# xitorch/xitorch

Measured on AMD Instinct MI355X. Metric: eigpairs/sec of symeig(davidson) + Lanczos-role matvec GB/s (roofline.achieved), batch=64 N=16384, higher is better.
Workload: dtype f64

## Files before the change

include/xitorch_amd.h:

```cpp
#ifndef XITORCH_AMD_H
#define XITORCH_AMD_H

#ifdef __cplusplus
extern "C" {
#endif

#define XK_OK 0
#define XK_ERR_ARG (-1)
#define XK_ERR_UNSUPPORTED (-2)

int xk_abi_version(void);

int xk_stream_read(const void* src, long bytes, long pitch_bytes, void* scratch, void* stream);
int xk_stream_create_cu_masked(int device, int reserve_cus, void** stream_out);
int xk_stream_create_cu_masked_pattern(int device, int reserve_cus, int pattern, void** stream_out);
int xk_probe_xcc(unsigned* hist16, unsigned* units128, int workgroups, int spin_cycles, void* stream);
int xk_stream_destroy(void* stream);

long xk_dense_mm_workspace_elems(int B, int M, int N, int P, int trans);
int xk_dense_mm_f64(const double* A, const double* X, double* Y, double* ws, long ws_elems,
                    int B, int M, int N, int P, long lda, long sA, long ldx, long sX,
                    long ldy, long sY, int trans, int rows_hint, int stagger, void* stream);
int xk_dense_mm_f32(const float* A, const float* X, float* Y, float* ws, long ws_elems,
                    int B, int M, int N, int P, long lda, long sA, long ldx, long sX,
// ... 2 lines not shown
long xk_dense_symm_workspace_elems(int B, int N, int P, int elem_size);
int xk_dense_symm_f64(const double* A, const double* X, double* Y, double* ws, long ws_elems, int B,
                      int N, int P, long lda, long sA, long ldx, long sX, long ldy, long sY, int opts, void* stream);
int xk_dense_symm_f32(const float* A, const float* X, float* Y, float* ws, long ws_elems, int B, int N,
                      int P, long lda, long sA, long ldx, long sX, long ldy, long sY, int opts, void* stream);
int xk_dense_symm_tiles_f64(const double* A, const double* X, double* ws, long ws_elems, int B, int N, int P,
                            long lda, long sA, long ldx, long sX, int opts, void* stream);
int xk_dense_symm_tiles_f32(const float* A, const float* X, float* ws, long ws_elems, int B, int N, int P,
                            long lda, long sA, long ldx, long sX, int opts, void* stream);
int xk_dense_symm_fold_f64(double* Y, const double* ws, long ws_elems, int B, int N, int P, long ldy, long sY,
                           int opts, void* stream);
int xk_dense_symm_fold_f32(float* Y, const float* ws, long ws_elems, int B, int N, int P, long ldy, long sY,
                           int opts, void* stream);

long xk_dense_symm_wide_workspace_elems(int B, int N);
int xk_dense_symm_wide_f32(const float* A, const float* X, float* Y, float* ws, long ws_elems, int B, int N, int P,
                           long lda, long sA, long ldx, long sX, long ldy, long sY, int opts, void* stream);
int xk_dense_symm_wide_tiles_f32(const float* A, const float* X, float* ws, long ws_elems, int B, int N, int P,
                                 long lda, long sA, long ldx, long sX, int opts, void* stream);
int xk_dense_symm_wide_fold_f32(float* Y, const float* ws, long ws_elems, int B, int N, int P, long ldy, long sY,
                                int opts, void* stream);

long xk_dense_wide_workspace_elems(int B, int M, int N, int P, int elem_size);
int xk_dense_wide_padded_width(int P, int elem_size);
int xk_dense_wide_f32(const float* A, const float* Xrm, float* Y, float* ws, long ws_elems, int B, int M,
                      int N, int P, long lda, long sA, long ldxr, long sXr, long ldy, long sY, void* stream);
int xk_dense_wide_f64(const double* A, const double* Xrm, double* Y, double* ws, long ws_elems, int B, int M,
                      int N, int P, long lda, long sA, long ldxr, long sXr, long ldy, long sY, void* stream);

long xk_dense_rows_wide_workspace_elems(int B, int M, int N, int P, int elem_size);
int xk_dense_rows_wide_f64(const double* A, const double* X, double* Y, double* ws, long ws_elems, int B, int M,
                           int N, int P, long lda, long sA, long ldx, long sX, long ldy, long sY, void* stream);
int xk_dense_rows_wide_f32(const float* A, const float* X, float* Y, float* ws, long ws_elems, int B, int M, int N,
                           int P, long lda, long sA, long ldx, long sX, long ldy, long sY, void* stream);

int xk_lincomb_f64(const double* V, const double* C, double* Out, int B, int k, int N, int P,
                   long ldv, long sV, long sC, long sCa, long sCc, long ldo, long sO,
                   double alpha, double beta, void* stream);
int xk_lincomb_f32(const float* V, const float* C, float* Out, int B, int k, int N, int P,
                   long ldv, long sV, long sC, long sCa, long sCc, long ldo, long sO,
                   double alpha, double beta, void* stream);
int xk_ritz_residual_f64(const double* V, const double* AV, const double* Y, const double* lam,
                         double* X, double* Tn, double* rmax, int B, int k, int N, int P,
                         long ldv, long sV, long ldav, long sAV, long sY, long sYa, long sYc,
                         long sLam, long ldx, long sX, long ldt, long sT, void* stream);
int xk_ritz_residual_f32(const float* V, const float* AV, const float* Y, const float* lam,
                         float* X, float* Tn, float* rmax, int B, int k, int N, int P,
                         long ldv, long sV, long ldav, long sAV, long sY, long sYa, long sYc,
                         long sLam, long ldx, long sX, long ldt, long sT, void* stream);
int xk_panel_chol_f64(const double* G, double* W, int* info, int B, int P, long ldg, long sG, void* stream);
int xk_panel_chol_f32(const float* G, float* W, int* info, int B, int P, long ldg, long sG, void* stream);
int xk_panel_transform_f64(double* Tp, const double* W, int B, int P, int N, long ldt, long sT, void* stream);
int xk_panel_transform_f32(float* Tp, const float* W, int B, int P, int N, long ldt, long sT, void* stream);

int xk_diag_precond_f64(double* t, const double* d, const double* m, const double* lam, int B, int N, int P,
                        long ldt, long sT, long sD, long sM, long sLam, double floor_, void* stream);
int xk_diag_precond_f32(float* t, const float* d, const float* m, const float* lam, int B, int N, int P,
                        long ldt, long sT, long sD, long sM, long sLam, double floor_, void* stream);

int xk_group_status_f64(const double* rmax, const int* info, const int* flag, double* orth, double* status, int B,
                        void* stream);
int xk_group_status_f32(const float* rmax, const int* info, const int* flag, float* orth, double* status, int B,
                        void* stream);

long xk_small_eigh_workspace_elems(int B, int k, int max_sweeps);
int xk_small_eigh_f64(const double* T, double* lam, double* Y, double* ws, long ws_elems, int* sweeps,
                      int B, int k, int p, int uppest, int max_sweeps, long ldt, long sT, void* stream);
int xk_small_eigh_f32(const float* T, float* lam, float* Y, float* ws, long ws_elems, int* sweeps,
                      int B, int k, int p, int uppest, int max_sweeps, long ldt, long sT, void* stream);

long xk_small_eigh_tri_lds_bytes(int k, int p, int elem_size);
int xk_small_eigh_tri_f64(const double* T, double* lam, double* Y, int* info, int B, int k, int p, int uppest,
                          long ldt, long sT, int threads, long long* profile, void* stream);
int xk_small_eigh_tri_f32(const float* T, float* lam, float* Y, int* info, int B, int k, int p, int uppest, long ldt,
                          long sT, int threads, long long* profile, void* stream);

int xk_banded_mm_f64(const double* band, const double* X, double* Y, int B, int N, int hb, int C,
                     long sBand, long ldx, long sX, long ldy, long sY, int trans, void* stream);
int xk_banded_mm_f32(const float* band, const float* X, float* Y, int B, int N, int hb, int C,
                     long sBand, long ldx, long sX, long ldy, long sY, int trans, void* stream);

int xk_csr_seg_len(void);
int xk_csr_mm_f64(const int* ptr, const int* idx, const int* perm, const double* val, long sV, const int* rows,
                  const int* bin_off, const int* seg_q, const int* seg_off, int nseg, double* ws, const double* X,
                  double* Y, int B, int Mout, int Nin, int C, long ldx, long sX, long ldy, long sY, void* stream);
int xk_csr_mm_f32(const int* ptr, const int* idx, const int* perm, const float* val, long sV, const int* rows,
                  const int* bin_off, const int* seg_q, const int* seg_off, int nseg, float* ws, const float* X,
                  float* Y, int B, int Mout, int Nin, int C, long ldx, long sX, long ldy, long sY, void* stream);
int xk_csr_sddmm_f64(const int* row_of, const int* col, const double* U, const double* W, double* G, int nnz, int B,
                     int M, int N, int C, long ldu, long sU, long ldw, long sW, long sG, void* stream);
int xk_csr_sddmm_f32(const int* row_of, const int* col, const float* U, const float* W, float* G, int nnz, int B,
                     int M, int N, int C, long ldu, long sU, long ldw, long sW, long sG, void* stream);
int xk_csr_mm_c128(const int* ptr, const int* idx, const int* perm, const double* val, long sV, const int* rows,
                   const int* bin_off, const int* seg_q, const int* seg_off, int nseg, double* ws, const double* X,
                   double* Y, int B, int Mout, int Nin, int C, long ldx, long sX, long ldy, long sY, int conj_val,
                   void* stream);
int xk_csr_mm_c64(const int* ptr, const int* idx, const int* perm, const float* val, long sV, const int* rows,
                  const int* bin_off, const int* seg_q, const int* seg_off, int nseg, float* ws, const float* X,
                  float* Y, int B, int Mout, int Nin, int C, long ldx, long sX, long ldy, long sY, int conj_val,
                  void* stream);
int xk_csr_sddmm_c128(const int* row_of, const int* col, const double* U, const double* W, double* G, int nnz, int B,
                      int M, int N, int C, long ldu, long sU, long ldw, long sW, long sG, void* stream);
int xk_csr_sddmm_c64(const int* row_of, const int* col, const float* U, const float* W, float* G, int nnz, int B,
                     int M, int N, int C, long ldu, long sU, long ldw, long sW, long sG, void* stream);

int xk_banded_grad_f64(const double* U, const double* W, double* G, int B, int N, int hb, int C, long ldu,
// ... 298 lines not shown
```

xitorch_amd/csrc/xk_basis.hip:

```cpp
#include "xk_common.h"

namespace xk {

template <typename T, int P>
__global__ __launch_bounds__(256) void lincomb_kernel(
    const T* __restrict__ V, const T* __restrict__ C, T* __restrict__ Out,
    int k, int N, long ldv, long sV, long sC, long sCa, long sCc, long ldo, long sO,
    T alpha, T beta, int col_tiles) {
  typedef typename Vec16<T>::type VT;
  constexpr int VN = Vec16<T>::n;
  const int b = blockIdx.x / col_tiles;
  const int ct = blockIdx.x - b * col_tiles;
  const int j = (ct * 256 + threadIdx.x) * VN;
  if (j >= N) return;
  const T* Vb = V + (long)b * sV + j;
  const T* Cb = C + (long)b * sC;
  VT acc[P];
#pragma unroll
  for (int c = 0; c < P; ++c)
#pragma unroll
    for (int v = 0; v < VN; ++v) acc[c][v] = T(0);
  int a = 0;
  for (; a + 8 <= k; a += 8) {
    VT v[8];
// ... 235 lines not shown
  constexpr int VN = Vec16<T>::n;
  if (!vec_ok<T>(N, ldv, sV, V) || !vec_ok<T>(N, ldo, sO, Out)) return XK_ERR_UNSUPPORTED;
  const int ct = (N + 256 * VN - 1) / (256 * VN);
  int c0 = 0;
  while (c0 < P) {
    const int pc = (P - c0) >= 8 ? 8 : (P - c0);
    const T* Cc = C + (long)c0 * sCc;
    T* Oc = Out + (long)c0 * ldo;
    switch (pc) {
#define XK_CASE(PP)                                                                                   \
  case PP:                                                                                            \
    hipLaunchKernelGGL((lincomb_kernel<T, PP>), dim3((unsigned)((long)B * ct)), dim3(256), 0, st, V, \
                       Cc, Oc, k, N, ldv, sV, sC, sCa, sCc, ldo, sO, alpha, beta, ct);                \
    break;
      XK_CASE(1) XK_CASE(2) XK_CASE(3) XK_CASE(4) XK_CASE(5) XK_CASE(6) XK_CASE(7) XK_CASE(8)
#undef XK_CASE
    }
    XK_LAUNCH_CHECK();
    c0 += pc;
  }
  return XK_OK;
}

template <typename T>
static int ritz_residual(const T* V, const T* AV, const T* Y, const T* lam, T* X, T* Tn, T* rmax, int B,
                         int k, int N, int P, long ldv, long sV, long ldav, long sAV, long sY, long sYa,
                         long sYc, long sLam, long ldx, long sX, long ldt, long sT, hipStream_t st) {
  constexpr int VN = Vec16<T>::n;
  if (!vec_ok<T>(N, ldv, sV, V) || !vec_ok<T>(N, ldav, sAV, AV) || !vec_ok<T>(N, ldx, sX, X) ||
      !vec_ok<T>(N, ldt, sT, Tn))
    return XK_ERR_UNSUPPORTED;
  const int ct = (N + 256 * VN - 1) / (256 * VN);
  int c0 = 0;
  while (c0 < P) {
    const int pc = (P - c0) >= 8 ? 8 : (P - c0);
    switch (pc) {
#define XK_CASE(PP)                                                                                    \
  case PP:                                                                                             \
    hipLaunchKernelGGL((ritz_residual_kernel<T, PP>), dim3((unsigned)((long)B * ct)), dim3(256), 0,   \
                       st, V, AV, Y + (long)c0 * sYc, lam + c0, X + (long)c0 * ldx, Tn + (long)c0 * ldt, \
                       rmax, k, N, ldv, sV, ldav, sAV, sY, sYa, sYc, sLam, ldx, sX, ldt, sT, ct);       \
    break;
      XK_CASE(1) XK_CASE(2) XK_CASE(3) XK_CASE(4) XK_CASE(5) XK_CASE(6) XK_CASE(7) XK_CASE(8)
#undef XK_CASE
    }
    XK_LAUNCH_CHECK();
    c0 += pc;
  }
  return XK_OK;
}


template <typename T>
__global__ __launch_bounds__(256) void diag_precond_kernel(T* __restrict__ Tn, const T* __restrict__ d,
                                                            const T* __restrict__ m, const T* __restrict__ lam,
                                                            int N, int P, long ldt, long sT, long sD, long sM,
                                                            long sLam, T floor_, long total) {
  const long idx = (long)blockIdx.x * 256 + threadIdx.x;
  if (idx >= total) return;
  const long per_b = (long)P * N;
  const long b = idx / per_b;
  const long rem = idx - b * per_b;
  const int c = (int)(rem / N);
  const int n = (int)(rem - (long)c * N);
  const T mm = m ? m[b * sM + n] : T(1);
  T den = d[b * sD + n] - lam[b * sLam + c] * mm;
  if (fabs(den) < floor_) den = den < T(0) ? -floor_ : floor_;
  T* t = Tn + b * sT + (long)c * ldt + n;
  *t = *t / den;
}

template <typename T>
__global__ __launch_bounds__(64) void group_status_kernel(const T* __restrict__ rmax, const int* __restrict__ info,
                                                          const int* __restrict__ flag, T* __restrict__ orth,
                                                          double* __restrict__ status, int B) {
  const int lane = threadIdx.x;
  double m = 0.0, om_ = 0.0;
  int nan = 0, i1 = 0, i2 = 0;
  bool first = true;
  for (int b = lane; b < B; b += 64) {
    const double v = (double)rmax[b];
    nan |= (v != v);
    m = first ? v : (v > m ? v : m);
    const int a = info[b];
    i1 = first ? a : (a > i1 ? a : i1);
    if (flag) {
      const int f = flag[b];
      i2 = first ? f : (f > i2 ? f : i2);
    }
    if (orth) {
      const double ov = (double)orth[b];
      orth[b] = T(0);
      om_ = (ov != ov) ? __builtin_inf() : (ov > om_ ? ov : om_);
    }
    first = false;
  }
  double mm = first ? -__builtin_inf() : m;
  int a1 = first ? -2147483647 - 1 : i1, a2 = first ? -2147483647 - 1 : i2;
#pragma unroll
  for (int sft = 32; sft >= 1; sft >>= 1) {
    const double om = __shfl_xor(mm, sft, 64), oo = __shfl_xor(om_, sft, 64);
    const int o1 = __shfl_xor(a1, sft, 64), o2 = __shfl_xor(a2, sft, 64), on = __shfl_xor(nan, sft, 64);
    mm = om > mm ? om : mm;
    om_ = oo > om_ ? oo : om_;
    a1 = o1 > a1 ? o1 : a1;
    a2 = o2 > a2 ? o2 : a2;
    nan |= on;
  }
  if (lane == 0) {
    status[0] = nan ? __builtin_nan("") : mm;
    status[1] = (double)a1;
    status[2] = flag ? (double)a2 : 0.0;
    if (orth) status[4] = om_;
  }
}

}

extern "C" {

#define XK_DEFINE_BASIS(SUF, T)                                                                          \
  int xk_lincomb_##SUF(const T* V, const T* C, T* Out, int B, int k, int N, int P, long ldv, long sV,    \
                       long sC, long sCa, long sCc, long ldo, long sO, double alpha, double beta,        \
                       void* stream) {                                                                   \
    if (B < 0 || k < 0 || N < 0 || P < 0) return XK_ERR_ARG;                                             \
    if (B == 0 || N == 0 || P == 0) return XK_OK;                                                        \
    return xk::lincomb<T>(V, C, Out, B, k, N, P, ldv, sV, sC, sCa, sCc, ldo, sO, (T)alpha, (T)beta,      \
                          (hipStream_t)stream);                                                          \
  }                                                                                                      \
  int xk_ritz_residual_##SUF(const T* V, const T* AV, const T* Y, const T* lam, T* X, T* Tn, T* rmax,    \
                             int B, int k, int N, int P, long ldv, long sV, long ldav, long sAV,         \
                             long sY, long sYa, long sYc, long sLam, long ldx, long sX, long ldt,        \
                             long sT, void* stream) {                                                    \
    if (B < 0 || k < 0 || N < 0 || P < 0) return XK_ERR_ARG;                                             \
    if (B == 0 || N == 0 || P == 0) return XK_OK;                                                        \
    return xk::ritz_residual<T>(V, AV, Y, lam, X, Tn, rmax, B, k, N, P, ldv, sV, ldav, sAV, sY, sYa,     \
                                sYc, sLam, ldx, sX, ldt, sT, (hipStream_t)stream);                       \
  }                                                                                                      \
  int xk_panel_chol_##SUF(const T* G, T* W, int* info, int B, int P, long ldg, long sG, void* stream) {  \
    if (B < 0 || P < 0 || P > 32) return XK_ERR_ARG;                                                     \
    if (B == 0 || P == 0) return XK_OK;                                                                  \
    hipLaunchKernelGGL((xk::panel_chol_kernel<T>), dim3((unsigned)B), dim3(64), 0,                       \
                       (hipStream_t)stream, G, W, info, B, P, ldg, sG, (long)P * P);                     \
    XK_LAUNCH_CHECK();                                                                                   \
    return XK_OK;                                                                                        \
  }                                                                                                      \
  int xk_panel_transform_##SUF(T* Tp, const T* W, int B, int P, int N, long ldt, long sT,                \
                               void* stream) {                                                           \
    if (B < 0 || P < 0 || N < 0) return XK_ERR_ARG;                                                      \
    if (B == 0 || P == 0 || N == 0) return XK_OK;                                                        \
    if (!xk::vec_ok<T>(N, ldt, sT, Tp)) return XK_ERR_UNSUPPORTED;                                       \
    constexpr int VN = xk::Vec16<T>::n;                                                                  \
    const int ct = (N + 256 * VN - 1) / (256 * VN);                                                      \
    hipLaunchKernelGGL((xk::panel_transform_kernel<T>), dim3((unsigned)((long)B * ct)), dim3(256), 0,    \
                       (hipStream_t)stream, Tp, W, P, N, ldt, sT, (long)P * P, ct);                      \
    XK_LAUNCH_CHECK();                                                                                   \
    return XK_OK;                                                                                        \
  }

XK_DEFINE_BASIS(f64, double)
XK_DEFINE_BASIS(f32, float)

#define XK_DEFINE_STATUS(SUF, T)                                                                            \
  int xk_group_status_##SUF(const T* rmax, const int* info, const int* flag, T* orth, double* status, int B, \
                            void* stream) {                                                                 \
    if (B <= 0 || !rmax || !info || !status) return XK_ERR_ARG;                                             \
    hipLaunchKernelGGL((xk::group_status_kernel<T>), dim3(1), dim3(64), 0, (hipStream_t)stream, rmax, info, \
                       flag, orth, status, B);                                                              \
    XK_LAUNCH_CHECK();                                                                                      \
    return XK_OK;                                                                                           \
  }
XK_DEFINE_STATUS(f64, double)
XK_DEFINE_STATUS(f32, float)

// ... 16 lines not shown
```

xitorch_amd/kernels.py:

```python
import os
import torch
from xitorch_amd import _capi
from xitorch_amd._capi import ptr, stream_ptr, check, suffix, fn, call, require_device
from ctypes import c_void_p as c_void_p_

__all__ = ["dense_mm"]


def _panel_strides(X):
    if X.dim() != 3 or (X.shape[-1] > 1 and X.stride(-1) != 1):
        raise _capi.NativeLibraryError("panel must be (B, P, N) with unit stride along N, got shape %s stride %s"
                                       % (tuple(X.shape), X.stride()))
    return X.stride(1), X.stride(0)


def _op_strides(A):
    if A.dim() == 2:
        return A.stride(0), 0
    return A.stride(1), (A.stride(0) if A.shape[0] != 1 else 0)


def _esize(dtype):
    return 8 if dtype == torch.float64 else 4

# ... 129 lines not shown
_gs_cache = {}


def _guard_scratch(B, P, dtype, device):
    key = (dtype, device, torch.cuda.current_stream().cuda_stream)
    g = _gs_cache.get(key)
    if g is None or g.numel() < B * P * P:
        g = _gs_cache[key] = torch.empty(B * P * P, dtype=dtype, device=device)
    return g


def _check_ritz_shapes(V, AV, Y, lam, X, Tn, k, P):
    B = V.shape[0]
    if Y.dim() != 3 or Y.shape[0] != B or Y.shape[1] < k or Y.shape[2] < P or lam.shape[0] != B or lam.shape[-1] < P:
        raise _capi.NativeLibraryError("ritz_residual: Y must be (B, >=k, >=P) and lam (B, >=P); got %s / %s for "
                                       "k = %d, P = %d" % (tuple(Y.shape), tuple(lam.shape), k, P))
    if V.shape[1] < k or AV.shape[1] < k or X.shape[1] < P or Tn.shape[1] < P:
        raise _capi.NativeLibraryError("ritz_residual: basis / output panels are smaller than (k, P) = (%d, %d)" % (k, P))


def ritz_residual(V, AV, Y, lam, X, Tn, rmax, k, P):
    B, N = V.shape[0], V.shape[2]
    if lam.stride(-1) != 1 and P > 1:
        raise _capi.NativeLibraryError("lam must have unit stride along its last dim")
    _check_ritz_shapes(V, AV, Y, lam, X, Tn, k, P)
    call("xk_ritz_residual", V.dtype, ptr(V), ptr(AV), ptr(Y), ptr(lam), ptr(X), ptr(Tn), ptr(rmax), B, k, N, P,
         V.stride(1), V.stride(0), AV.stride(1), AV.stride(0), Y.stride(0), Y.stride(1), Y.stride(2), lam.stride(0),
         X.stride(1), X.stride(0), Tn.stride(1), Tn.stride(0))


def diag_precond(Tn, d, lam, P, m=None, floor=None):
    B, N = Tn.shape[0], d.shape[-1]
    if floor is None:
        floor = float(torch.finfo(Tn.dtype).eps) ** 0.5
    d2 = d.reshape(-1, N)
    m2 = m.reshape(-1, N) if m is not None else None
    for t in (d2, m2):
        if t is not None and (t.stride(-1) != 1 or t.dtype != Tn.dtype or t.shape[0] not in (1, B)):
            raise _capi.NativeLibraryError("diag_precond: diagonals must be (B or 1, N), unit stride, dtype of the panel")
    sD = d2.stride(0) if d2.shape[0] == B and B > 1 else (0 if d2.shape[0] == 1 else d2.stride(0))
    sM = 0 if m2 is None or m2.shape[0] == 1 else m2.stride(0)
    call("xk_diag_precond", Tn.dtype, ptr(Tn), ptr(d2), ptr(m2) if m2 is not None else None, ptr(lam), B, N, P,
         Tn.stride(1), Tn.stride(0), sD, sM, lam.stride(0), float(floor))


def panel_chol(G, W, info, P):
    B = G.shape[0]
    call("xk_panel_chol", G.dtype, ptr(G), ptr(W), ptr(info), B, P, G.stride(1), G.stride(0))


def panel_transform(Tp, W, P):
    B, N = Tp.shape[0], Tp.shape[2]
    call("xk_panel_transform", Tp.dtype, ptr(Tp), ptr(W), B, P, N, Tp.stride(1), Tp.stride(0))


def davidson_ritz(V, AV, Y, lam, X, Tn, rmax, info, flag, status, k, P, cond=None, orth=None):
    B, N = V.shape[0], V.shape[2]
    if lam.stride(-1) != 1 and P > 1:
        raise _capi.NativeLibraryError("lam must have unit stride along its last dim")
    _check_ritz_shapes(V, AV, Y, lam, X, Tn, k, P)
    gs, ws, nws = None, None, 0
    if orth is not None:
        if status.numel() < 5:
            raise _capi.NativeLibraryError("davidson_ritz: status needs 5 doubles when orth is given")
        if P > 8:
            gs = _guard_scratch(B, P, V.dtype, V.device)
            nws = fn("xk_dense_mm_workspace_elems")(B, P, N, P, 0)
            ws = _workspace(max(nws, 1), V.dtype, V.device)
    call("xk_davidson_ritz", V.dtype, ptr(V), ptr(AV), ptr(Y), ptr(lam), ptr(X), ptr(Tn), ptr(rmax), ptr(info),
         ptr(flag) if flag is not None else None, ptr(cond) if cond is not None else None,
         ptr(orth) if orth is not None else None, ptr(status), B, k, N, P, V.stride(1), V.stride(0), AV.stride(1),
         AV.stride(0), Y.stride(0), Y.stride(1), Y.stride(2), lam.stride(0), X.stride(1), X.stride(0), Tn.stride(1),
         Tn.stride(0), ptr(gs), (gs.numel() if gs is not None else 0), ptr(ws), nws)


def davidson_ws(B, cap, N, q, dtype, device):
    nws = fn("xk_dense_mm_workspace_elems")(B, cap, N, q, 0)
    return _workspace(max(nws, 1), dtype, device), nws


def davidson_orth(V, N, k0, q, C, W, info, passes=2, cond=None):
    B = V.shape[0]
    ws, nws = davidson_ws(B, V.shape[1], N, q, V.dtype, V.device)
    call("xk_davidson_orth", V.dtype, ptr(V), B, N, k0, q, V.stride(1), V.stride(0), ptr(C), ptr(W), ptr(info),
         ptr(cond) if cond is not None else None, ptr(ws), nws, int(passes))


def davidson_extend_t(V, AV, Tm, Tn, N, k0, q):
    B = V.shape[0]
    ws, nws = davidson_ws(B, V.shape[1], N, q, V.dtype, V.device)
    call("xk_davidson_extend_t", V.dtype, ptr(V), ptr(AV), ptr(Tm), ptr(Tn), B, N, k0, q, V.stride(1), V.stride(0),
         AV.stride(1), AV.stride(0), Tm.stride(1), Tm.stride(0), ptr(ws), nws)


SMALL_EIGH_MAX_K = 128
SMALL_EIGH_MAX_P = 16


SMALL_EIGH_TRI_MIN_K = 16


def small_eigh_tri_ok(k, p, dtype):
    if k > SMALL_EIGH_MAX_K or p > SMALL_EIGH_MAX_P or p > k:
        return False
    return fn("xk_small_eigh_tri_lds_bytes")(k, p, _esize(dtype)) <= 160 * 1024

# ... 848 lines not shown
```

xitorch_amd/linalg/native_eig.py:

```python
import os
import torch
from xitorch_amd import kernels as K
from xitorch_amd._capi import NativeLibraryError
from xitorch_amd._util import bcast_shape
from xitorch_amd.linalg._panel import PanelOperator, pad_len, batch_count, require_hip
from xitorch_amd.dist import allreduce_max_

__all__ = ["davidson", "exacteig", "take_eigpairs", "tallqr_extend", "native_partial_eigh"]

_PRELAUNCH = True
CHAIN_CUS = "all"
K3G_MAX_K = [1536, 1024]
K3P_MIN_K = int(os.environ.get("XITORCH_K3P_MIN_K", "80"))


def take_eigpairs(evals, evecs, neig, mode):
    if mode == "lowest":
        return evals[..., :neig], evecs[..., :neig]
    return evals[..., -neig:], evecs[..., -neig:]


def _shift_rel(N, q, rdtype):
    u = torch.finfo(rdtype).eps * 0.5
    return min(11.0 * (N * q + q * (q + 1)) * u, 1e-3)


def _gram(Vrows, k, panel, p, N):
    return K.dense_mm(Vrows[:, :k, :N], panel[:, :p, :N])


def _shard_of_global_batch(B, device, process_group):
    world = torch.distributed.get_world_size(process_group)
    rank = torch.distributed.get_rank(process_group)
    mine = torch.tensor([float(B)], dtype=torch.float64, device=device)
    allb = [torch.zeros_like(mine) for _ in range(world)]
    torch.distributed.all_gather(allb, mine, group=process_group)
    counts = [int(round(v.item())) for v in allb]
    return sum(counts[:rank]), sum(counts)


def _initial_block(v_init, V0, bdims, B, N, nguess, dtype, device, rng_device="cpu", shard=None):
    if V0 is not None:
        if V0.shape[-2] != N:
            raise RuntimeError("V0 must have shape (*batch, %d, nguess), got %s" % (N, tuple(V0.shape)))
        V = V0.to(device=device, dtype=dtype).expand(*bdims, N, V0.shape[-1]).reshape(B, N, V0.shape[-1])
        return V.transpose(-2, -1)
    kind = v_init.lower()
    if kind == "cos":
        from xitorch_amd import synthetic
        return synthetic.start_block(B, N, nguess, dtype, device)
    torch.manual_seed(12421)
    rdev = torch.device("cpu") if rng_device == "cpu" else device
    if kind == "eye":
        V = torch.eye(N, nguess, dtype=dtype, device=rdev).unsqueeze(0).repeat(B, 1, 1)
    elif kind in ("randn", "rand", "random"):
        draw = torch.randn if kind == "randn" else torch.rand
        if shard is not None and shard[1] != B:
            off, total = shard
            V = draw((total, N, nguess), dtype=dtype, device=rdev)[off:off + B].clone()
        else:
            V = draw((*bdims, N, nguess), dtype=dtype, device=rdev).reshape(B, N, nguess)
    else:
        raise ValueError("Unknown v_init type: %s" % kind)
    return V.to(device).transpose(-2, -1)


class _Group:

    def __init__(self, opA, opM, B, N, Npad, p, nguess, dtype, device, mode, small_eigh, orth_passes,
                 precond=None, restart=None, capacity=None):
        self.opA, self.opM = opA, opM
        self.precond = precond
        self.restart = restart
        self.keep = 2 * p
        self._compress = None
        self.nrestart = 0
        self.k1_stream = None
        self.k1_sched = None
        self.pg = None
        self.timeline, self.tag = None, 0
        self.B, self.N, self.Npad, self.p = B, N, Npad, p
        self.dtype, self.device, self.mode = dtype, device, mode
        self.small_eigh, self.orth_passes = small_eigh, orth_passes
        self.nguess0 = nguess
        if restart is not None:
            want = restart + p
        elif capacity is not None:
            want = int(capacity)
        else:
            want = nguess + 8 * p
        self.cap = max(nguess, min(N, want)) if N > nguess else nguess
        z = lambda *shape: torch.zeros(shape, dtype=dtype, device=device)
        self.Vs, self.AVs = z(B, self.cap, Npad), z(B, self.cap, Npad)
        self.MVs = z(B, self.cap, Npad) if opM is not None else None
        self.T = z(B, self.cap, self.cap)
        self.Wflat = torch.empty((B * 32 * 32,), dtype=dtype, device=device)
        self._cscratch = None
        self.info = torch.zeros((B,), dtype=torch.int32, device=device)
        self.status = torch.zeros((5,), dtype=torch.float64, device=device)
        self.cond = torch.zeros((B,), dtype=dtype, device=device)
        self.orth = torch.zeros((B,), dtype=dtype, device=device)
        self.MXtmp = z(B, p, Npad) if opM is not None else None
        self.adaptive = False
        self.passes_now = 2
        self.two_pass_from = None
        self.rmax = z(B)
        self.Xbuf = [z(B, p, Npad), z(B, p, Npad)]
        self.k = 0
        self.fast = True
        self.best_slot, self.best_evals = -1, None
        self.slot, self.lam, self.newpanel, self.nadd = 0, None, None, 0

    def grow(self, need):
        if need <= self.cap:
            return
        new = min(self.N, max(need, 2 * self.cap))

        def bigger(old):
            buf = torch.zeros((self.B, new, self.Npad), dtype=self.dtype, device=self.device)
            buf[:, :old.shape[1]].copy_(old)
            return buf
        self.Vs, self.AVs = bigger(self.Vs), bigger(self.AVs)
        if self.MVs is not None:
            self.MVs = bigger(self.MVs)
        Tn = torch.zeros((self.B, new, new), dtype=self.dtype, device=self.device)
        Tn[:, :self.cap, :self.cap].copy_(self.T)
        self.T, self.cap = Tn, new

    def scratch(self, q):
        n = self.B * max(q, self.p) * (self.cap + q)
        if self._cscratch is None or self._cscratch.numel() < n:
            self._cscratch = torch.empty((n,), dtype=self.dtype, device=self.device)
        return self._cscratch

    def cholqr(self, k0, q, shifted=False):
        N = self.N
        if self.opM is None and self.fast and not shifted:
            K.davidson_orth(self.Vs, N, k0, q, self.scratch(q), self.Wflat, self.info, passes=0)
            return
        panel = self.Vs[:, k0:k0 + q]
        if self.opM is None:
            G = K.dense_mm(panel[:, :, :N], panel[:, :, :N])
        else:
            self.opM.apply(panel, self.MVs[:, k0:k0 + q])
            G = K.dense_mm(panel[:, :, :N], self.MVs[:, k0:k0 + q, :N])
        if shifted:
            sh = _shift_rel(N, q, self.dtype)
            tr = torch.diagonal(G, dim1=-2, dim2=-1).sum(-1)
            G = G + (sh * tr)[:, None, None] * torch.eye(q, dtype=G.dtype, device=G.device)
        Wq = self.Wflat[:self.B * q * q].view(self.B, q, q)
        K.panel_chol(G, Wq, self.info, q)
        K.panel_transform(panel, Wq, q)
        if self.opM is not None:
            K.panel_transform(self.MVs[:, k0:k0 + q], Wq, q)

    def project_out(self, k0, q):
        panel = self.Vs[:, k0:k0 + q]
        basis_for_coef = self.Vs if self.opM is None else self.MVs
        C = _gram(basis_for_coef, k0, panel, q, self.N)
        K.lincomb(self.Vs, C, panel, k0, q, coef_layout="ca", alpha=-1.0, beta=1.0)

    def extend_T(self, k0, q):
        N = self.N
        if self.fast:
            K.davidson_extend_t(self.Vs, self.AVs, self.T, self.scratch(q), N, k0, q)
            return
        Tn = K.dense_mm(self.Vs[:, :k0 + q, :N], self.AVs[:, k0:k0 + q, :N])
        self.T[:, k0:k0 + q, :k0 + q] = Tn
        self.T[:, :k0, k0:k0 + q] = Tn[:, :, :k0].transpose(-2, -1)

    def _mark(self, label, stream=None):
        if self.timeline is None:
            return lambda: None
        st = stream if stream is not None else torch.cuda.current_stream()
        e0 = torch.cuda.Event(enable_timing=True)
        e0.record(st)

# ... 33 lines not shown
        tri_flag = None
        self._orth_done = False
        due = self.restart is not None and k + p > self.restart and k > self.keep and k < N
        pk = min(self.keep, k) if due else p
        self._compress = None
        tri_fits = K.small_eigh_tri_ok(k, p, self.dtype) and K.small_eigh_tri_ok(k, pk, self.dtype)
        prefer_big = self.small_eigh == "native" and not force_jacobi and k <= K.SMALL_EIGH_MAX_K and \
            pk <= K.SMALL_EIGH_MAX_P and ((k >= K3P_MIN_K and getattr(self, "chain_exposed", False)) or
                                          (k >= K.SMALL_EIGH_TRI_MIN_K and not tri_fits)) and \
            K.small_eigh_big_ok(k, pk, self.dtype)
        if self.small_eigh in ("native", "jacobi", "tri") and k <= K.SMALL_EIGH_MAX_K and pk <= K.SMALL_EIGH_MAX_P \
                and not prefer_big:
            end = self._mark("k3")
            use_tri = (not force_jacobi) and self.small_eigh != "jacobi" and \
                (k >= K.SMALL_EIGH_TRI_MIN_K or self.small_eigh == "tri") and K.small_eigh_tri_ok(k, p, self.dtype)
            use_tri = use_tri and K.small_eigh_tri_ok(k, pk, self.dtype)
            if use_tri:
                lam, Yt, tri_flag = K.small_eigh(self.T, k, pk, uppest=(self.mode != "lowest"), method="tri")
            else:
                lam, Yt, _ = K.small_eigh(self.T, k, pk, uppest=(self.mode != "lowest"))
            end()
            if due:
                self._compress = (Yt, lam)
                sl = slice(0, p) if self.mode == "lowest" else slice(pk - p, pk)
                lam, Yt = lam[:, sl].contiguous(), Yt[:, sl]
            Y = Yt.transpose(1, 2)
        elif self.small_eigh in ("native", "tri") and not force_jacobi and \
                (k > K.SMALL_EIGH_MAX_K or pk > K.SMALL_EIGH_MAX_P or prefer_big) and \
                k <= K3G_MAX_K[0 if self.B >= 16 else 1] and K.small_eigh_big_ok(k, pk, self.dtype):
            end = self._mark("k3")
            lam, Yt, tri_flag = K.small_eigh_big(self.T, k, pk, uppest=(self.mode != "lowest"))
            end()
            if due:
                self._compress = (Yt, lam)
                sl = slice(0, p) if self.mode == "lowest" else slice(pk - p, pk)
                lam, Yt = lam[:, sl].contiguous(), Yt[:, sl]
            Y = Yt.transpose(1, 2)
        else:
            lam_all, Y_all = torch.linalg.eigh(self.T[:, :k, :k])
            if due:
                lk, Yk = take_eigpairs(lam_all, Y_all, pk, self.mode)
                self._compress = (Yk.transpose(1, 2).contiguous(), lk.contiguous())
            lam, Y = take_eigpairs(lam_all, Y_all, p, self.mode)
            lam = lam.contiguous()
        end_ritz = self._mark("ritz")
        self.grow(min(N, k + p))
        self.nadd = min(p, N - k)
        self.slot = 1 - self.best_slot if self.best_slot >= 0 else 0
        X = self.Xbuf[self.slot]
        if not (self.fast and self.opM is None and self.precond is None):
            self.rmax.zero_()
        if self.nadd == p and not due:
            self.newpanel = self.Vs[:, k:k + p]
        else:
            self.newpanel = torch.empty((self.B, p, self.Npad), dtype=self.dtype, device=self.device)
        fused_status = self.fast and self.opM is None and self.precond is None
        if fused_status:
            K.davidson_ritz(self.Vs, self.AVs, Y, lam, X, self.newpanel, self.rmax, self.info, tri_flag, self.status,
                            k, p, cond=self.cond, orth=self.orth)
        elif self.opM is None:
            K.ritz_residual(self.Vs, self.AVs, Y, lam, X, self.newpanel, self.rmax, k, p)
            K.ritz_guard(X, self.orth, p, self.Npad)
        else:
            K.ritz_residual(self.MVs, self.AVs, Y, lam, self.MXtmp, self.newpanel, self.rmax, k, p)
            K.lincomb(self.Vs, Y, X, k, p, coef_layout="ac", alpha=1.0, beta=0.0)
            K.ritz_guard(X, self.orth, p, self.Npad, MX=self.MXtmp)
        if self.precond is not None:
            if self.precond[0] == "diag":
                K.diag_precond(self.newpanel, self.precond[1], lam, p, m=self.precond[2])
            else:
                tmp = torch.zeros_like(self.newpanel)
                self.precond[1].apply(self.newpanel, tmp)
                self.newpanel.copy_(tmp)
        self.lam = lam
        if not fused_status:
            K.group_status(self.rmax, self.info, tri_flag, self.status, orth=self.orth)
        if self.pg is not None:
            torch.nan_to_num_(self.status, nan=float("inf"), posinf=float("inf"))
            allreduce_max_(self.status, self.pg)
        end_ritz()

    def compress(self):
        Yt, lam_all = self._compress
        self._compress = None
        k, pk = self.k, Yt.shape[1]
        for name in ("Vs", "AVs", "MVs"):
            buf = getattr(self, name)
            if buf is None:
                continue
            tmp = torch.zeros((self.B, pk, self.Npad), dtype=self.dtype, device=self.device)
            K.lincomb(buf, Yt, tmp, k, pk, coef_layout="ca", alpha=1.0, beta=0.0)
            buf[:, :pk].copy_(tmp)
        self.T.zero_()
        self.T[:, :pk, :pk] = torch.diag_embed(lam_all)
        K.ritz_guard(self.Vs, self.orth, pk, self.Npad, MX=self.MVs)
        self.k = pk
        self.nrestart += 1

    def rollback(self, k_good, passes):
        self.k = k_good
        self._compress = None
        self._orth_done = False
        self.adaptive = False
        self.orth_passes = max(int(self.orth_passes), int(passes))
        self.info.zero_()
        self.cond.zero_()
        self.orth.zero_()
        self.reorthonormalise(k_good)

    def reorthonormalise(self, k):
        N, B = self.N, self.B
        bufs = [b for b in (self.Vs, self.AVs, self.MVs) if b is not None]
        coef_basis = self.Vs if self.opM is None else self.MVs
        k0 = 0
        while k0 < k:
            q = min(self.p if k0 > 0 else max(self.nguess0, 1), 32, k - k0)
            panel = self.Vs[:, k0:k0 + q]
            for it in range(2):
                if k0 > 0:
                    C = _gram(coef_basis, k0, panel, q, N)
                    for buf in bufs:
                        K.lincomb(buf, C, buf[:, k0:k0 + q], k0, q, coef_layout="ca", alpha=-1.0, beta=1.0)
                Mp = panel if self.opM is None else self.MVs[:, k0:k0 + q]
                G = K.dense_mm(panel[:, :, :N], Mp[:, :, :N])
                G = (G + G.transpose(1, 2)) * 0.5
                if it == 0:
                    sh = _shift_rel(N, q, self.dtype)
                    tr = torch.diagonal(G, dim1=-2, dim2=-1).sum(-1)
                    G = G + (sh * tr)[:, None, None] * torch.eye(q, dtype=G.dtype, device=G.device)
                Wq = torch.empty((B, q, q), dtype=self.dtype, device=self.device)
                K.panel_chol(G.contiguous(), Wq, self.info, q)
                for buf in bufs:
                    K.panel_transform(buf[:, k0:k0 + q], Wq, q)
            k0 += q
        Tn = K.dense_mm(self.Vs[:, :k, :N], self.AVs[:, :k, :N], wide=False)
        self.T[:, :k, :k] = (Tn + Tn.transpose(1, 2)) * 0.5

    def expand_orth(self):
        restarted = self._compress is not None
        if restarted:
            self.compress()
        k, nadd = self.k, self.nadd
        if nadd != self.p or restarted:
            self.Vs[:, k:k + nadd].copy_(self.newpanel[:, :nadd])
        end = self._mark("orth")
        if self.fast and self.opM is None:
            K.davidson_orth(self.Vs, self.N, k, nadd, self.scratch(nadd), self.Wflat, self.info,
                            passes=self.current_passes(nadd), cond=self.cond)
        else:
            rounds = self.current_passes(nadd)
            for it in range(rounds):
                self.project_out(k, nadd)
                if rounds >= 2 or it == rounds - 1:
                    self.cholqr(k, nadd, shifted=(rounds >= 2 and it == 0))
        end()
        self._orth_done = True

    ONE_PASS_MAX_COND2 = 1e4

    def current_passes(self, q):
        if not self.adaptive:
            return max(1, self.orth_passes)
        if q > 8 or not (self.fast and self.opM is None and self.precond is None):
            return 2
        return self.passes_now

    def note_condition(self, cond2, it):
        limit = self.ONE_PASS_MAX_COND2 if self.dtype == torch.float64 else min(self.ONE_PASS_MAX_COND2, 1e2)
        if self.adaptive and self.passes_now == 1 and not (cond2 <= limit):
            self.passes_now = 2
            self.two_pass_from = it
        elif self.adaptive and self.two_pass_from is None and self.passes_now == 2 and cond2 <= limit and it >= 1:
            self.passes_now = 1

    def distrust(self, it):
        if self.adaptive and self.passes_now == 1:
            self.passes_now = 2
        if self.adaptive and self.two_pass_from is None:
            self.two_pass_from = it

    def speculate_orth(self):
        if self._compress is None and self.nadd > 0 and self.k < self.N:
            self.expand_orth()

    def expand_apply(self):
        k, nadd = self.k, self.nadd
        self.apply_A(self.Vs[:, k:k + nadd], self.AVs[:, k:k + nadd])
        end = self._mark("extT")
        self.extend_T(k, nadd)
        end()
        self.k = k + nadd
        self._orth_done = False

    def expand(self):
        if not getattr(self, "_orth_done", False):
            self.expand_orth()
        self.expand_apply()


def tallqr_extend(V, t, M=None, orth_passes=2):
    B, N, k = V.shape
    p = t.shape[-1]
    dev, dtype = V.device, V.dtype
    opM = PanelOperator(M, [B], B, N) if M is not None else None
    grp = _Group(None, opM, B, N, pad_len(N), p, k, dtype, dev, "lowest", "native", orth_passes)
    grp.grow(k + p)
    grp.Vs[:, :k, :N].copy_(V.transpose(-2, -1))
    grp.Vs[:, k:k + p, :N].copy_(t.transpose(-2, -1))
    if opM is not None:
        opM.apply(grp.Vs[:, :k], grp.MVs[:, :k])
    rounds = max(1, orth_passes)
    for it in range(rounds):
        grp.project_out(k, p)
        if rounds >= 2 or it == rounds - 1:
            grp.cholqr(k, p, shifted=(rounds >= 2 and it == 0))
    if int(grp.info.max().item()) != 0:
        raise RuntimeError("xitorch_amd tallqr_extend: the panel Gram matrix is not positive definite "
                           "(linearly dependent vectors)")
    return grp.Vs[:, :k + p, :N].transpose(-2, -1)


def _sub_operator(A, B, N, b0, b1):
    from xitorch_amd.linop import MatrixLinearOperator
    mat = A.mat.reshape(B, N, N)[b0:b1]
    sub = MatrixLinearOperator(mat, A.is_hermitian, symmetric_storage=getattr(A, "symmetric_storage", False))
    if getattr(A, "hermitian_verified", False):
        from xitorch_amd.linop import _storage_token
        sub._herm_token = _storage_token(mat)
    return sub


class _GuardFailure(RuntimeError):
    """the a-posteriori guard failed and the run cannot be rolled back to a basis that passed it"""


GUARD_GOOD = {torch.float64: 1e-10, torch.float32: 5e-5}
GUARD_BAD = {torch.float64: 1e-8, torch.float32: 5e-4}
GUARD_MAX_REDO = 3


def davidson(A, neig, mode, M=None, max_niter=1000, nguess=None, v_init="randn", max_addition=None,
             min_eps=1e-6, verbose=False, V0=None, orth_passes="auto", process_group=None, trace=None,
             rng_device="cpu", small_eigh="native", overlap="auto", precond=None, reserve_cus="auto", restart=None,
             groups="auto", chain="calls", basis_capacity=None, **unused):
# ... 292 lines not shown
                        groups[gg].expand()
                deferred = []
            else:
                deferred.append(g)
        max_resid = local_max
        policy.seen(guard, groups[0].nrestart)
        if policy.void(bad, guard):
            k_to, passes = policy.roll_back(bad, guard, k_rr, niter, trace)
            for g in range(G):
                with torch.cuda.stream(streams[g]):
                    groups[g].rollback(k_to, passes)
            history.append(max_resid)
            if verbose:
                print("Iter %3d (guess size: %d): guard %.2e: back to %d vectors" % (it + 1, k_rr, guard, k_to))
            continue
        if not policy.passed(guard, k_rr):
            for grp in groups:
                grp.distrust(it)
        history.append(max_resid)
        if verbose:
            print("Iter %3d (guess size: %d): resid: %.3e" % (it + 1, k_rr, max_resid))
        if max_resid < best_resid:
            best_resid = max_resid
            for grp in groups:
                grp.best_slot, grp.best_evals = grp.slot, grp.lam
        if max_resid < min_eps:
            stop_reason = "converged"
            break
        if k_rr == N:
            stop_reason = "full_basis"
            break
        for g in deferred:
            with torch.cuda.stream(streams[g]):
                groups[g].expand()

    if groups[0].best_slot < 0:
        raise RuntimeError("xitorch_amd davidson: no finite residual was produced")
    if two:
        cur = torch.cuda.current_stream()
        for st in streams + list(set(k1_streams)) + [t for (_, sts) in (k1_sched or []) for t in sts]:
            cur.wait_stream(st)
        evals = torch.cat([grp.best_evals for grp in groups], dim=0)
        Xall = torch.cat([grp.Xbuf[grp.best_slot] for grp in groups], dim=0)
        for grp in groups:
            grp.best_evals.record_stream(cur)
            grp.Xbuf[grp.best_slot].record_stream(cur)
    else:
        evals, Xall = groups[0].best_evals, groups[0].Xbuf[groups[0].best_slot]
    if trace is not None:
        trace.update(niter=niter, napply=sum(op.napply for op in ops) // G, resid_history=history,
                     basis_size=groups[0].k, best_resid=best_resid, stop_reason=stop_reason, groups=G,
                     k3_fallbacks=n_fallback[0], restarts=groups[0].nrestart, panel_kernel=ops[0].last_kernel,
                     orth_two_pass_from=[grp.two_pass_from for grp in groups], orth_adaptive=bool(adaptive),
                     orth_cond2_history=cond_hist, orth_guard_history=guard_hist, orth_redo=redo)
    evals = evals.reshape(*bdims, p)
    evecs = Xall[:, :, :N].transpose(-2, -1).reshape(*bdims, N, p)
    return evals, evecs


davidson.__doc__ = _davidson.__doc__ + "\n    (" + davidson.__doc__ + ")\n"


EXACTEIG_NATIVE_MAX_N = K.SMALL_EIGH_BIG_MAX_K
EXACTEIG_NATIVE_MAX_P = K.SMALL_EIGH_BIG_MAX_P


def _native_dense_ok(mat, neig):
    n = mat.shape[-1]
    nb = mat.numel() // max(1, n * n)
    return (mat.is_cuda and mat.dtype in (torch.float64, torch.float32) and 8 <= n <= EXACTEIG_NATIVE_MAX_N
            and n <= K3G_MAX_K[0 if nb >= 16 else 1]
            and 1 <= neig <= min(EXACTEIG_NATIVE_MAX_P, n) and mat.numel() > 0
            and K.small_eigh_big_ok(n, neig, mat.dtype))


def native_partial_eigh(mat, neig, mode):
    bdims, n = mat.shape[:-2], mat.shape[-1]
    T = mat.reshape(-1, n, n)
    if T.stride(-1) != 1:
        T = T.contiguous()
    upp = (mode != "lowest")
    if n <= K.SMALL_EIGH_MAX_K and neig <= K.SMALL_EIGH_MAX_P and n >= K.SMALL_EIGH_TRI_MIN_K and \
            K.small_eigh_tri_ok(n, neig, T.dtype):
        lam, Yt, flag = K.small_eigh(T, n, neig, uppest=upp, method="tri")
    else:
        lam, Yt, flag = K.small_eigh_big(T, n, neig, uppest=upp)
    X = Yt.transpose(1, 2)
    if int(flag.max().item()) != 0:
        bad = torch.nonzero(flag, as_tuple=False).flatten()
        l2, U2 = torch.linalg.eigh(T[bad])
        l2, U2 = take_eigpairs(l2, U2, neig, mode)
        lam = lam.clone()
        X = X.clone()
        lam[bad], X[bad] = l2, U2
    return lam.reshape(*bdims, neig), X.reshape(*bdims, n, neig)


class _NativeEigh(torch.autograd.Function):

    @staticmethod
    def forward(ctx, A, neig, mode):
        lam, X = native_partial_eigh(A.detach(), neig, mode)
        ctx.save_for_backward(A, X)
        ctx.neig, ctx.mode = neig, mode
        return lam, X

    @staticmethod
# ... 74 lines not shown
```

Baseline: 1808.

## Size Davidson basis from operator footprint and grow it copying only live rows

Adds a heuristic that picks the first basis capacity from the operator's memory footprint, allocating room for many more blocks when the basis is small relative to the operator. This avoids repeated regrowth of the basis during the run. When the basis does grow, a new HIP kernel copies only the live rows into an uninitialized buffer and zero-fills the rest, replacing a full zero-fill plus copy. The cost is a possibly larger up-front allocation, plus extra bookkeeping of pending rows that rollback and orth paths must keep correct.

```diff
diff --git a/include/xitorch_amd.h b/include/xitorch_amd.h
--- a/include/xitorch_amd.h
+++ b/include/xitorch_amd.h
@@ -78,6 +78,10 @@
 int xk_panel_chol_f32(const float* G, float* W, int* info, int B, int P, long ldg, long sG, void* stream);
 int xk_panel_transform_f64(double* Tp, const double* W, int B, int P, int N, long ldt, long sT, void* stream);
 int xk_panel_transform_f32(float* Tp, const float* W, int B, int P, int N, long ldt, long sT, void* stream);
+int xk_basis_grow_f64(const double* src, double* dst, int B, int live_rows, int dst_rows, int N, long ld_src,
+                      long s_src, long ld_dst, long s_dst, void* stream);
+int xk_basis_grow_f32(const float* src, float* dst, int B, int live_rows, int dst_rows, int N, long ld_src,
+                      long s_src, long ld_dst, long s_dst, void* stream);
 
 int xk_diag_precond_f64(double* t, const double* d, const double* m, const double* lam, int B, int N, int P,
                         long ldt, long sT, long sD, long sM, long sLam, double floor_, void* stream);
diff --git a/xitorch_amd/csrc/xk_basis.hip b/xitorch_amd/csrc/xk_basis.hip
--- a/xitorch_amd/csrc/xk_basis.hip
+++ b/xitorch_amd/csrc/xk_basis.hip
@@ -311,6 +311,32 @@
 
 
 template <typename T>
+__global__ __launch_bounds__(256) void basis_grow_kernel(const T* __restrict__ src, T* __restrict__ dst,
+                                                         int live_rows, int dst_rows, int nvec, long lds, long sS,
+                                                         long ldd, long sD, int col_tiles, int row_tiles) {
+  typedef typename Vec16<T>::type VT;
+  constexpr int VN = Vec16<T>::n;
+  const int ct = blockIdx.x % col_tiles;
+  const int rb = blockIdx.x / col_tiles;
+  const int rt = rb % row_tiles;
+  const int b = rb / row_tiles;
+  const long j = ((long)ct * 256 + threadIdx.x) * VN;
+  if (j >= ldd) return;
+  const int r0 = rt * 4;
+  VT v[4];
+#pragma unroll
+  for (int u = 0; u < 4; ++u) {
+#pragma unroll
+    for (int e = 0; e < VN; ++e) v[u][e] = T(0);
+    if (r0 + u < live_rows && j < nvec)
+      v[u] = *reinterpret_cast<const VT*>(src + (long)b * sS + (long)(r0 + u) * lds + j);
+  }
+#pragma unroll
+  for (int u = 0; u < 4; ++u)
+    if (r0 + u < dst_rows) *reinterpret_cast<VT*>(dst + (long)b * sD + (long)(r0 + u) * ldd + j) = v[u];
+}
+
+template <typename T>
 __global__ __launch_bounds__(256) void diag_precond_kernel(T* __restrict__ Tn, const T* __restrict__ d,
                                                             const T* __restrict__ m, const T* __restrict__ lam,
                                                             int N, int P, long ldt, long sT, long sD, long sM,
@@ -374,11 +400,42 @@
   }
 }
 
+template <typename T>
+static int basis_grow(const T* src, T* dst, int B, int live_rows, int dst_rows, int N, long lds, long sS, long ldd,
+                      long sD, hipStream_t st) {
+  constexpr int VN = Vec16<T>::n;
+  const long nvec = ((long)N + VN - 1) / VN * VN;
+  if (!vec_ok<T>(N, ldd, sD, dst) || ldd < nvec) return XK_ERR_UNSUPPORTED;
+  if (live_rows > 0 && (!vec_ok<T>(N, lds, sS, src) || lds < nvec)) return XK_ERR_UNSUPPORTED;
+  if (sS < 0 || (B > 1 && sD < (long)dst_rows * ldd)) return XK_ERR_ARG;
+  if (ldd == 0) return XK_OK;
+  const long ct = (ldd + 256 * VN - 1) / (256 * VN);
+  const long rt = ((long)dst_rows + 3) / 4;
+  const long blocks = (long)B * rt * ct;
+  if (blocks > 2147483647L) return XK_ERR_UNSUPPORTED;
+  hipLaunchKernelGGL((basis_grow_kernel<T>), dim3((unsigned)blocks), dim3(256), 0, st, src, dst, live_rows, dst_rows,
+                     (int)nvec, lds, sS, ldd, sD, (int)ct, (int)rt);
+  XK_LAUNCH_CHECK();
+  return XK_OK;
+}
+
 }
 
 extern "C" {
 
-#define XK_DEFINE_BASIS(SUF, T)                                                                          \
+#define XK_DEFINE_GROW(SUF, T)                                                                           \
+  int xk_basis_grow_##SUF(const T* src, T* dst, int B, int live_rows, int dst_rows, int N, long ld_src,  \
+                          long s_src, long ld_dst, long s_dst, void* stream) {                           \
+    if (B < 0 || live_rows < 0 || dst_rows < live_rows || N < 0) return XK_ERR_ARG;                      \
+    if (B == 0 || dst_rows == 0) return XK_OK;                                                           \
+    if (!dst || (live_rows > 0 && !src)) return XK_ERR_ARG;                                              \
+    return xk::basis_grow<T>(src, dst, B, live_rows, dst_rows, N, ld_src, s_src, ld_dst, s_dst,          \
+                             (hipStream_t)stream);                                                       \
+  }
+XK_DEFINE_GROW(f64, double)
+XK_DEFINE_GROW(f32, float)
+
+#define XK_DEFINE_BASIS(SUF, T)                                                                         \
   int xk_lincomb_##SUF(const T* V, const T* C, T* Out, int B, int k, int N, int P, long ldv, long sV,    \
                        long sC, long sCa, long sCc, long ldo, long sO, double alpha, double beta,        \
                        void* stream) {                                                                   \
diff --git a/xitorch_amd/kernels.py b/xitorch_amd/kernels.py
--- a/xitorch_amd/kernels.py
+++ b/xitorch_amd/kernels.py
@@ -205,6 +205,22 @@
 def panel_transform(Tp, W, P):
     B, N = Tp.shape[0], Tp.shape[2]
     call("xk_panel_transform", Tp.dtype, ptr(Tp), ptr(W), B, P, N, Tp.stride(1), Tp.stride(0))
+
+
+def basis_grow(src, dst, live_rows, N, raw=False):
+    require_device(dst, "basis buffer")
+    if dst.dim() != 3 or (src is not None and (src.dim() != 3 or src.dtype != dst.dtype or src.shape[0] != dst.shape[0])):
+        raise _capi.NativeLibraryError("basis_grow: (B, rows, ld) buffers of one dtype and batch expected")
+    if dst.shape[2] > 1 and (dst.stride(2) != 1 or (src is not None and src.stride(2) != 1)):
+        raise _capi.NativeLibraryError("basis_grow: unit stride along the vector axis expected")
+    if live_rows > 0 and (src is None or src.shape[1] < live_rows or src.shape[2] < N):
+        raise _capi.NativeLibraryError("basis_grow: the source holds fewer than %d rows of length %d" % (live_rows, N))
+    if dst.shape[2] != dst.stride(1) or dst.shape[2] < N:
+        raise _capi.NativeLibraryError("basis_grow: the destination's rows must be whole pitches of at least N elements")
+    B, dst_rows = dst.shape[0], dst.shape[1]
+    lds, sS = (src.stride(1), src.stride(0)) if src is not None else (dst.stride(1), 0)
+    return call("xk_basis_grow", dst.dtype, ptr(src), ptr(dst), B, live_rows, dst_rows, N, lds, sS, dst.stride(1),
+                dst.stride(0), raw=raw)
 
 
 def davidson_ritz(V, AV, Y, lam, X, Tn, rmax, info, flag, status, k, P, cond=None, orth=None):
diff --git a/xitorch_amd/linalg/native_eig.py b/xitorch_amd/linalg/native_eig.py
--- a/xitorch_amd/linalg/native_eig.py
+++ b/xitorch_amd/linalg/native_eig.py
@@ -6,7 +6,7 @@
 from xitorch_amd.linalg._panel import PanelOperator, pad_len, batch_count, require_hip
 from xitorch_amd.dist import allreduce_max_
 
-__all__ = ["davidson", "exacteig", "take_eigpairs", "tallqr_extend", "native_partial_eigh"]
+__all__ = ["davidson", "exacteig", "take_eigpairs", "tallqr_extend", "native_partial_eigh", "first_capacity"]
 
 _PRELAUNCH = True
 CHAIN_CUS = "all"
@@ -65,6 +65,33 @@
     return V.to(device).transpose(-2, -1)
 
 
+FIRST_CAPACITY_BLOCKS = 20
+FIRST_CAPACITY_SHARE = 32
+
+
+def first_capacity(N, nguess, neig, basis_row_bytes, operator_bytes, basis_capacity=None, restart=None):
+    if restart is not None:
+        return int(restart) + neig
+    if basis_capacity is not None:
+        return int(basis_capacity)
+    clamp = lambda rows: max(nguess, min(N, rows))
+    roomy = clamp(nguess + FIRST_CAPACITY_BLOCKS * neig)
+    if 2 * roomy * basis_row_bytes * FIRST_CAPACITY_SHARE <= operator_bytes:
+        return roomy
+    return clamp(nguess + 8 * neig)
+
+
+def _operator_bytes(op):
+    kind = getattr(op, "kind", "generic")
+    if kind == "dense":
+        return op.mat.numel() * op.mat.element_size()
+    if kind == "banded":
+        return op.band.numel() * op.band.element_size()
+    if kind == "csr":
+        return op.vals.numel() * (op.vals.element_size() + 4)
+    return 0
+
+
 class _Group:
 
     def __init__(self, opA, opM, B, N, Npad, p, nguess, dtype, device, mode, small_eigh, orth_passes,
@@ -83,17 +110,18 @@
         self.dtype, self.device, self.mode = dtype, device, mode
         self.small_eigh, self.orth_passes = small_eigh, orth_passes
         self.nguess0 = nguess
-        if restart is not None:
-            want = restart + p
-        elif capacity is not None:
-            want = int(capacity)
-        else:
-            want = nguess + 8 * p
+        esize = torch.empty((), dtype=dtype).element_size()
+        want = first_capacity(N, nguess, p, B * Npad * esize, _operator_bytes(opA), basis_capacity=capacity,
+                              restart=restart)
         self.cap = max(nguess, min(N, want)) if N > nguess else nguess
         z = lambda *shape: torch.zeros(shape, dtype=dtype, device=device)
         self.Vs, self.AVs = z(B, self.cap, Npad), z(B, self.cap, Npad)
         self.MVs = z(B, self.cap, Npad) if opM is not None else None
         self.T = z(B, self.cap, self.cap)
+        self.row_bytes = B * Npad * esize * (2 if opM is None else 3)
+        self.alloc_bytes = self.cap * self.row_bytes
+        self.growth = []
+        self.pending = 0
         self.Wflat = torch.empty((B * 32 * 32,), dtype=dtype, device=device)
         self._cscratch = None
         self.info = torch.zeros((B,), dtype=torch.int32, device=device)
@@ -115,14 +143,16 @@
         if need <= self.cap:
             return
         new = min(self.N, max(need, 2 * self.cap))
+        live = min(self.cap, self.k + self.pending)
 
         def bigger(old):
-            buf = torch.zeros((self.B, new, self.Npad), dtype=self.dtype, device=self.device)
-            buf[:, :old.shape[1]].copy_(old)
+            buf = torch.empty((self.B, new, self.Npad), dtype=self.dtype, device=self.device)
+            K.basis_grow(old, buf, live, self.N)
             return buf
         self.Vs, self.AVs = bigger(self.Vs), bigger(self.AVs)
         if self.MVs is not None:
             self.MVs = bigger(self.MVs)
+        self.growth.append((self.cap, new, new * self.row_bytes, live * self.row_bytes))
         Tn = torch.zeros((self.B, new, new), dtype=self.dtype, device=self.device)
         Tn[:, :self.cap, :self.cap].copy_(self.T)
         self.T, self.cap = Tn, new
@@ -262,7 +292,9 @@
             self.rmax.zero_()
         if self.nadd == p and not due:
             self.newpanel = self.Vs[:, k:k + p]
+            self.pending = p
         else:
+            self.pending = 0
             self.newpanel = torch.empty((self.B, p, self.Npad), dtype=self.dtype, device=self.device)
         fused_status = self.fast and self.opM is None and self.precond is None
         if fused_status:
@@ -309,6 +341,7 @@
 
     def rollback(self, k_good, passes):
         self.k = k_good
+        self.pending = 0
         self._compress = None
         self._orth_done = False
         self.adaptive = False
@@ -353,6 +386,7 @@
         k, nadd = self.k, self.nadd
         if nadd != self.p or restarted:
             self.Vs[:, k:k + nadd].copy_(self.newpanel[:, :nadd])
+            self.pending = nadd
         end = self._mark("orth")
         if self.fast and self.opM is None:
             K.davidson_orth(self.Vs, self.N, k, nadd, self.scratch(nadd), self.Wflat, self.info,
@@ -400,6 +434,7 @@
         self.extend_T(k, nadd)
         end()
         self.k = k + nadd
+        self.pending = 0
         self._orth_done = False
 
     def expand(self):
@@ -798,7 +833,9 @@
                      basis_size=groups[0].k, best_resid=best_resid, stop_reason=stop_reason, groups=G,
                      k3_fallbacks=n_fallback[0], restarts=groups[0].nrestart, panel_kernel=ops[0].last_kernel,
                      orth_two_pass_from=[grp.two_pass_from for grp in groups], orth_adaptive=bool(adaptive),
-                     orth_cond2_history=cond_hist, orth_guard_history=guard_hist, orth_redo=redo)
+                     orth_cond2_history=cond_hist, orth_guard_history=guard_hist, orth_redo=redo,
+                     basis_alloc_bytes=sum(grp.alloc_bytes for grp in groups),
+                     basis_growth=[ev for grp in groups for ev in grp.growth])
     evals = evals.reshape(*bdims, p)
     evecs = Xall[:, :, :N].transpose(-2, -1).reshape(*bdims, N, p)
     return evals, evecs
```

Result: no change. 1859 (median of 3 runs) (+2.8%).
